# sndels/prosper

Measured on AMD Instinct MI355X. Metric: Mpaths/s, higher is better.
Workload: dtype f32; 1 GPU; S-cornell 1920x1080 8spp maxBounces 4; width=1920, height=1080, spp=8, max_bounces=4, triangles=38, bvh_nodes=7, parallelism=image stripes x1, pipeline=wavefront, 3 frames in flight (one launch chain each)

## Files before the change

### include/prosper_pt/prosper_pt.h

```cpp
#ifndef PROSPER_PT_H
#define PROSPER_PT_H

#include <stddef.h>
#include <stdint.h>

#include "shader_structs.h"

#ifdef __cplusplus
extern "C" {
#endif

#define PROSPER_PT_ABI_VERSION 4

enum
{
    PROSPER_PT_OK = 0,
    PROSPER_PT_ERR_INVALID_ARGUMENT = -1,
    PROSPER_PT_ERR_NO_DEVICE = -2,
    PROSPER_PT_ERR_HIP = -3,
    PROSPER_PT_ERR_NO_SCENE = -4,
    PROSPER_PT_ERR_SCENE = -5,
    PROSPER_PT_ERR_UNSUPPORTED = -6,
    PROSPER_PT_NOT_READY = -7,
};
// ... 119 lines not shown
    uint64_t pixelsWritten;
    uint64_t historyReads;
    uint64_t shortIndexHits;
    uint64_t shortIndexTriangleTests;
    uint64_t nodePhaseSteps;
    uint64_t trianglePhaseSteps;
    uint64_t anyHitTexelFetches;
} prosper_pt_counters;

typedef struct prosper_pt_scene_stats
{
    uint64_t triangleCount;
    uint64_t nodeCount;
    uint32_t nodeBytes;
    uint32_t triangleBytes;
    uint32_t maxDepth;
    uint32_t variantFlags;
    uint64_t deviceBytes;
    double buildSeconds;
    double uploadSeconds;
    double bvhBuildSeconds;
    double textureSeconds;
    uint64_t alphaTriangleCount;
    uint64_t alphaBoundBytes;
} prosper_pt_scene_stats;
enum
{
    PROSPER_PT_VARIANT_LDS_SCENE = 1u << 0,
    PROSPER_PT_VARIANT_LDS_TABLES = 1u << 1,
    PROSPER_PT_VARIANT_BATCHED_TEXTURES = 1u << 2,
    PROSPER_PT_VARIANT_TEXTURE_PACKS = 1u << 3,
    PROSPER_PT_VARIANT_RAW_RECORDS = 1u << 4,
    PROSPER_PT_VARIANT_STACK_SHIFT = 8,
};

enum
{
    PROSPER_PT_RENDER_COUNT_WORK = 1u << 0,
    PROSPER_PT_RENDER_PIPELINED = 1u << 1,
};

typedef struct prosper_pt_debug_options
{
    uint32_t struct_size;
    int32_t batchedTextures;
    int32_t widePacks;
    int32_t alphaCellShift;
    uint32_t noTexturePacks;
    uint32_t noAlphaBounds;
    uint32_t noUploadRefit;
    uint32_t flatBvh;
    float sahTraversalCost;
    float boxPad;
    uint32_t leafSize;
    uint32_t buildThreads;
    uint32_t topEntries;
    int32_t nodeOrder;
    int32_t childOrder;
    uint32_t buildTiming;
    uint32_t segments;
    uint32_t segmentLength;
    uint32_t chains;
    uint32_t ldsStackEntries;
    uint32_t noLdsScene;
    uint32_t noLdsTables;
    uint32_t traceDeadPaths;
    int32_t bandedBatches;
    float rebuildCostRatio;
    uint32_t alwaysRebuild;
    uint32_t failNextUpdate;
    uint32_t poolVariant;
    uint32_t rawRecords;
    uint32_t tileOrder;
    uint32_t hipGraph;
    uint32_t pipelinedChains;
    uint32_t mergeLimit;
} prosper_pt_debug_options;

const char *prosper_pt_last_error(void);
uint32_t prosper_pt_abi_version(void);
uint32_t prosper_pt_has_experiments(void);
void prosper_pt_debug_options_default(prosper_pt_debug_options *out);
int prosper_pt_set_debug_options(prosper_pt_ctx *ctx, const prosper_pt_debug_options *options);
int prosper_pt_get_debug_options(prosper_pt_ctx *ctx, prosper_pt_debug_options *out);

int prosper_pt_create(const prosper_pt_device_desc *desc, prosper_pt_ctx **out_ctx);
void prosper_pt_destroy(prosper_pt_ctx *ctx);

int prosper_pt_upload_scene(prosper_pt_ctx *ctx, const prosper_pt_scene_view *scene);
int prosper_pt_update_lights(
    prosper_pt_ctx *ctx, const prosper_DirectionalLightParameters *directionalLight,
    const prosper_PointLightsBuffer *pointLights, const prosper_SpotLightsBuffer *spotLights);
int prosper_pt_update_transforms(prosper_pt_ctx *ctx, const prosper_ModelInstanceTransforms *transforms, uint32_t count);
enum
{
    PROSPER_PT_UPDATE_NOW = 1u << 0,
};
int prosper_pt_update_transforms_async(
    prosper_pt_ctx *ctx, const prosper_ModelInstanceTransforms *transforms, uint32_t count, uint32_t flags, void *stream);
#define PROSPER_PT_ANIMATION_NONE 0xFFFFFFFFu
enum
{
    PROSPER_PT_NODE_HAS_TRANSLATION = 1u << 0,
    PROSPER_PT_NODE_HAS_ROTATION = 1u << 1,
    PROSPER_PT_NODE_HAS_SCALE = 1u << 2,
    PROSPER_PT_NODE_DIRECTIONAL_LIGHT = 1u << 3,
    PROSPER_PT_NODE_CAMERA = 1u << 4,
};
enum
{
    PROSPER_PT_ANIMATION_PATH_TRANSLATION = 0,
    PROSPER_PT_ANIMATION_PATH_ROTATION = 1,
    PROSPER_PT_ANIMATION_PATH_SCALE = 2,
};
enum
{
    PROSPER_PT_ANIMATION_STEP = 0,
// ... 706 lines not shown
```

### prosper_amd/capi.py

```python
import ctypes as C
import os
import subprocess

import numpy as np

from . import structs as S

_HERE = os.path.dirname(os.path.abspath(__file__))
LIB_PATH = os.environ.get("PROSPER_PT_LIB") or os.path.join(_HERE, "libprosper_pt.so")


class ProsperPtError(RuntimeError):
    def __init__(self, code, message):
        super().__init__("prosper_pt error %d: %s" % (code, message))
        self.code = code


def build(force=False):
    args = ["make", "-C", os.path.join(_HERE, "csrc"), "-s"]
    if force:
        args.append("-B")
    subprocess.check_call(args)
    return LIB_PATH


_lib = None


def lib():
    global _lib
    if _lib is not None:
        return _lib
    if not os.path.exists(LIB_PATH):
        raise ProsperPtError(-2, "HIP extension %s is missing: run prosper_amd.capi.build()" % LIB_PATH)
    L = C.CDLL(LIB_PATH)
    vp, u32, i32 = C.c_void_p, C.c_uint32, C.c_int32
    L.prosper_pt_last_error.restype = C.c_char_p
    L.prosper_pt_abi_version.restype = u32
    L.prosper_pt_has_experiments.restype = u32
    L.prosper_pt_debug_options_default.argtypes = [C.POINTER(S.DebugOptions)]
    L.prosper_pt_debug_options_default.restype = None
    L.prosper_pt_set_debug_options.argtypes = [vp, C.POINTER(S.DebugOptions)]
    L.prosper_pt_get_debug_options.argtypes = [vp, C.POINTER(S.DebugOptions)]
    L.prosper_pt_create.argtypes = [C.POINTER(S.DeviceDesc), C.POINTER(vp)]
    L.prosper_pt_destroy.argtypes = [vp]
    L.prosper_pt_destroy.restype = None
    L.prosper_pt_upload_scene.argtypes = [vp, C.POINTER(S.SceneView)]
    L.prosper_pt_update_lights.argtypes = [
        vp, C.POINTER(S.DirectionalLightParameters), C.POINTER(S.PointLightsBuffer), C.POINTER(S.SpotLightsBuffer)]
    L.prosper_pt_get_scene_stats.argtypes = [vp, C.POINTER(S.SceneStats)]
    L.prosper_pt_update_textures.argtypes = [vp, vp, u32, u32]
    L.prosper_pt_update_materials.argtypes = [vp, vp, u32, u32]
    L.prosper_pt_texture_mip_level_count.argtypes = [u32, u32]
    L.prosper_pt_texture_mip_level_count.restype = u32
    L.prosper_pt_check_texture_desc.argtypes = [C.POINTER(S.TextureDesc), u32]
    L.prosper_pt_get_texture_mips_info.argtypes = [vp, u32, C.POINTER(S.TextureMipsInfo)]
    L.prosper_pt_read_texture_level.argtypes = [vp, u32, u32, vp, C.c_uint64, vp]
    L.prosper_pt_debug_sample_texture_lod.argtypes = [vp, u32, u32, vp, u32, C.c_float, vp]
    L.prosper_pt_set_texture_lod.argtypes = [vp, C.c_int, C.c_float]
    L.prosper_pt_set_texture_lod_debug.argtypes = [vp, C.c_int]
    L.prosper_pt_read_texture_lod_derivatives.argtypes = [vp, vp, C.c_size_t, vp]
    L.prosper_pt_update_meshes.argtypes = [vp, vp, u32]
    L.prosper_pt_finish_mesh_updates.argtypes = [vp]
    L.prosper_pt_update_transforms.argtypes = [vp, vp, u32]
    L.prosper_pt_update_transforms_async.argtypes = [vp, vp, u32, u32, vp]
    L.prosper_pt_set_animations.argtypes = [vp, C.POINTER(S.AnimationDesc)]
    L.prosper_pt_animate.argtypes = [vp, C.c_float, u32, vp]
    L.prosper_pt_get_animation_state.argtypes = [vp, C.POINTER(S.AnimationStateInfo)]
    L.prosper_pt_read_animated_transforms.argtypes = [vp, u32, vp, u32]
    L.prosper_pt_read_lights.argtypes = [
        vp, C.POINTER(S.DirectionalLightParameters), C.POINTER(S.PointLightsBuffer), C.POINTER(S.SpotLightsBuffer)]
    L.prosper_pt_debug_read_animation_nodes.argtypes = [vp, vp, vp, u32]
    L.prosper_pt_rebuild_hierarchy.argtypes = [vp]
    L.prosper_pt_get_hierarchy_state.argtypes = [vp, C.POINTER(S.HierarchyState)]
    L.prosper_pt_debug_read_nodes.argtypes = [vp, vp, C.c_size_t]
    L.prosper_pt_set_output_buffer.argtypes = [vp, vp, C.c_size_t]
# ... 331 lines not shown
    rg, b = np.empty(2 * half_width, np.float32), np.empty(2 * half_width, np.float32)
    lib().prosper_pt_bloom_streak_weights(half_width, rg.ctypes.data, b.ctypes.data)
    return rg, b


def bloom_fft_plan(width, height, resolution_scale=0):
    plan = S.BloomFftPlan()
    _check(lib().prosper_pt_bloom_fft_plan(width, height, resolution_scale, C.byref(plan)))
    return plan


def has_experiments():
    return bool(lib().prosper_pt_has_experiments())


_debug_defaults = {}
_debug_version = 0


def debug(**options):
    global _debug_version
    if not options:
        _debug_defaults.clear()
    for k, v in options.items():
        if k not in dict(S.DebugOptions._fields_):
            raise KeyError("unknown debug option %r" % k)
        if v is None:
            _debug_defaults.pop(k, None)
        else:
            _debug_defaults[k] = v
    _debug_version += 1


class Context:

    def __init__(self, device=0, flags=0, _borrowed=None):
        self._owned = _borrowed is None
        self._own_debug = {}
        self._base_debug = None
        self._debug_seen = -1
        self._world = None
        self._animation_nodes = 0
        self._restir_extent = None
        if _borrowed is not None:
            self._h = C.c_void_p(_borrowed)
            return
        desc = S.DeviceDesc(C.sizeof(S.DeviceDesc), device, flags, 0)
        h = C.c_void_p()
        _check(lib().prosper_pt_create(C.byref(desc), C.byref(h)))
        self._h = h

    def set_debug(self, **options):
        if not options:
            self._own_debug = {}
        for k, v in options.items():
            if k not in dict(S.DebugOptions._fields_):
                raise KeyError("unknown debug option %r" % k)
            if v is None:
                self._own_debug.pop(k, None)
            else:
                self._own_debug[k] = v
        self._debug_seen = -1
        self._sync_debug()

    def debug_options(self):
        o = S.DebugOptions()
# ... 834 lines not shown
```

### prosper_amd/csrc/prosper_pt.cpp

```cpp
#include "../../include/prosper_pt/prosper_pt.h"

#include <hip/hip_runtime.h>

#include <algorithm>
#include <chrono>
#include <future>
#include <memory>
#include <cmath>
#include <cstdlib>
#include <cstdio>
#include <cstring>
#include <exception>
#include <stdexcept>
#include <string>
#include <vector>

#include "bvh_build.hpp"
#include "pt_animation.hpp"
#include "pt_context.hpp"
#include "pt_geometry.hpp"
#include "pt_kernels.hpp"
#include "pt_materials.hpp"
#include "pt_pass_support.hpp"
#include "pt_scene.hpp"
// ... 51 lines not shown
    if (bytes) PPT_HIP(hipMemcpy(*out, src, bytes, hipMemcpyHostToDevice));
    return PROSPER_PT_OK;
}

int grow_buffer(DeviceBuffer &buf, GrowWait wait, hipStream_t s, size_t bytes, size_t allocBytes, int fill)
{
    hipError_t e = hipSuccess;
    if (wait == GrowWait::Stream) e = hipStreamSynchronize(s);
    if (wait == GrowWait::Device) e = hipDeviceSynchronize();
    if (buf.ptr)
    {
        const hipError_t f = hipFree(buf.ptr);
        if (e == hipSuccess) e = f;
    }
    buf.ptr = nullptr;
    buf.bytes = 0;
    if (e == hipSuccess) e = hipMalloc(&buf.ptr, allocBytes);
    if (e == hipSuccess && fill >= 0) e = hipMemset(buf.ptr, fill, allocBytes);
    if (e != hipSuccess)
    {
        if (buf.ptr) (void)hipFree(buf.ptr);
        buf.ptr = nullptr;
        return fail(PROSPER_PT_ERR_HIP, std::string("growing a device buffer: ") + hipGetErrorString(e));
    }
    buf.bytes = bytes;
    return PROSPER_PT_OK;
}

}

namespace
{

WavefrontOptions wavefront_options(const prosper_pt_ctx *ctx)
{
    const prosper_pt_debug_options &d = ctx->debug;
    WavefrontOptions o;
    o.ldsStackEntries = d.ldsStackEntries;
    o.noLdsScene = d.noLdsScene != 0;
    o.noLdsTables = d.noLdsTables != 0;
    return o;
}

}

namespace
{

void free_scene(prosper_pt_ctx *ctx)
{
    discard_mesh_build(ctx);
    for (ppt::AccelState *old : ctx->retiredAccel) delete old;
    ctx->retiredAccel.clear();
    for (auto &a : ctx->sceneAllocations) (void)hipFree(a.ptr);
    ctx->sceneAllocations.clear();
    delete ctx->accel;
    ctx->accel = nullptr;
    delete ctx->lights;
    ctx->lights = nullptr;
    delete ctx->materialState;
    ctx->materialState = nullptr;
    delete ctx->geometry;
    ctx->geometry = nullptr;
    ctx->dTransforms = nullptr;
    ctx->sceneBytes = 0;
    ctx->haveScene = false;
    ctx->scene = DeviceScene{};
    ctx->textureMips = nullptr;
}

int validate_scene(const prosper_pt_scene_view *v, bool mips)
{
    if (v->struct_size != sizeof(prosper_pt_scene_view))
        return fail(PROSPER_PT_ERR_INVALID_ARGUMENT, "scene view struct_size mismatch");
    if (v->geometryBufferCount && (!v->geometryBuffers || !v->geometryBufferByteSizes))
// ... 1081 lines not shown
    out->nodeCount = acc->nodeCount;
    out->levels = (uint32_t)acc->levelOffsets.size() - 1u;
    return PROSPER_PT_OK;
}

int prosper_pt_debug_read_nodes(prosper_pt_ctx *ctx, void *out, size_t byte_size)
{
    if (!ctx || !out) return fail(PROSPER_PT_ERR_INVALID_ARGUMENT, "prosper_pt_debug_read_nodes: null argument");
    if (!ctx->haveScene || !ctx->accel) return fail(PROSPER_PT_ERR_NO_SCENE, "no scene uploaded");
    const size_t bytes = (size_t)ctx->accel->nodeCount * sizeof(BvhNode);
    if (byte_size < bytes) return fail(PROSPER_PT_ERR_INVALID_ARGUMENT, "prosper_pt_debug_read_nodes: destination too small");
    PPT_HIP(hipSetDevice(ctx->device));
    {
        const int frc = flush_pending_update(ctx, nullptr);
        if (frc != PROSPER_PT_OK) return frc;
    }
    PPT_HIP(hipDeviceSynchronize());
    PPT_HIP(hipMemcpy(out, ctx->accel->dNodes, bytes, hipMemcpyDeviceToHost));
    return PROSPER_PT_OK;
}

int prosper_pt_get_scene_stats(prosper_pt_ctx *ctx, prosper_pt_scene_stats *out)
{
    if (!ctx || !out) return fail(PROSPER_PT_ERR_INVALID_ARGUMENT, "prosper_pt_get_scene_stats: null argument");
    if (!ctx->haveScene) return fail(PROSPER_PT_ERR_NO_SCENE, "no scene uploaded");
    *out = ctx->stats;
    const WavefrontPlan plan = wavefront_plan(
        ctx->stats.maxDepth, (uint32_t)ctx->stats.nodeCount, (uint32_t)ctx->stats.triangleCount, ctx->scene, wavefront_options(ctx));
    const uint32_t ldsEntries = plan.ldsStackEntries;
    out->variantFlags =
        (plan.sceneInLds ? PROSPER_PT_VARIANT_LDS_SCENE : 0u) | (plan.tablesInLds ? PROSPER_PT_VARIANT_LDS_TABLES : 0u) |
        (ctx->scene.batchedTextures ? PROSPER_PT_VARIANT_BATCHED_TEXTURES : 0u) |
        (ctx->packedMaterials ? PROSPER_PT_VARIANT_TEXTURE_PACKS : 0u) |
        (ldsEntries << PROSPER_PT_VARIANT_STACK_SHIFT);
    return PROSPER_PT_OK;
}

int prosper_pt_set_output_buffer(prosper_pt_ctx *ctx, void *device_rgba32f, size_t byte_size)
{
    if (!ctx) return fail(PROSPER_PT_ERR_INVALID_ARGUMENT, "prosper_pt_set_output_buffer: null context");
    if (device_rgba32f && (reinterpret_cast<uintptr_t>(device_rgba32f) & 15u))
        return fail(PROSPER_PT_ERR_INVALID_ARGUMENT, "output buffer must be 16-byte aligned");
    ctx->externalHdr = device_rgba32f;
    ctx->externalHdrBytes = device_rgba32f ? byte_size : 0;
    return PROSPER_PT_OK;
}

static int render_wavefront(
    prosper_pt_ctx *ctx, const RenderParams &p, bool countWork, bool pipelined, uint32_t slotIndex, LaunchTimeline *tp,
    hipStream_t s)
{
    const uint32_t tilesX = (p.localWidth + 7u) / 8u, tilesY = (p.height + 7u) / 8u;
    const uint64_t pixelsPadded = (uint64_t)tilesX * tilesY * 64u;
    constexpr uint64_t kMaxWavefrontSlots = 64ull << 20;
    if (pixelsPadded > kMaxWavefrontSlots) return fail(PROSPER_PT_ERR_UNSUPPORTED, "image too large for the wavefront workspace");
    uint32_t framesPerChunk = (uint32_t)(kMaxWavefrontSlots / pixelsPadded);
    if (framesPerChunk > p.frameCount) framesPerChunk = p.frameCount;
    RenderSlot &slot = ctx->slots[slotIndex];
    ctx->lastSlot = slotIndex;
    WavefrontChains chains;
    chains.count = (pipelined || (ctx->flags & PROSPER_PT_CREATE_SINGLE_CHAIN)) ? 1u : 2u;
    if (!pipelined && ctx->debug.chains >= 1u && ctx->debug.chains <= kMaxChains) chains.count = ctx->debug.chains;
    chains.detached = pipelined;
    chains.fork = &ctx->chainFork;
    for (uint32_t i = 0; i < kMaxChains; ++i)
    {
        chains.streams[i] = ctx->workStreams[pipelined ? slotIndex : i].get();
// ... 351 lines not shown
```

### prosper_amd/csrc/pt_kernels.hpp

```cpp
#pragma once

#include <hip/hip_runtime.h>

#include "pt_scene.hpp"
#include "pt_sync.hpp"

namespace ppt
{

enum : uint32_t
{
    kStageGenerate = 0,
    kStageShade = 1,
    kStageTrace = 2,
    kStageAccumulate = 3,
    kStageCount = 4,
};

void launch_flatten_triangles(
    const DeviceScene &s, const uint32_t *triOffsets, uint32_t drawInstanceCount, const uint32_t *drawInstanceFlags,
    WorldTriangle *out, ShadeTriangle *shadeOut, AlphaTriangle *alphaOut, uint32_t total, hipStream_t stream,
    const uint32_t *leafPosition = nullptr, WorldTriangle *leafOrder = nullptr);
void launch_refit(
    BvhNode *nodes, const WorldTriangle *tris, float4 *bounds, const uint32_t *order, const uint32_t *levelOffsets,
// ... 2 lines not shown
    const DeviceTexture &tex, uint32_t wrapS, uint32_t wrapT, float factorA, uint32_t shift, uint16_t *out, hipStream_t stream);
void launch_srgb_monotonicity(uint32_t firstBits, uint32_t lastBits, uint32_t *out, hipStream_t stream);
void launch_permute_triangles(
    const WorldTriangle *in, const uint32_t *permutation, WorldTriangle *out, uint32_t total, hipStream_t stream);
void launch_tone_map(
    const float4 *hdr, const uint32_t *lut, uint32_t dim, float exposure, float contrast, void *outRgba8, uint32_t count,
    hipStream_t stream);
uint32_t megakernel_grid_blocks(const RenderParams &p);
uint32_t wavefront_grid_blocks(const WavefrontBuffers &w);
void launch_render_megakernel(
    const DeviceScene &s, const RenderParams &p, float4 *hdr, unsigned long long *counters, int32_t *stackOverflow,
    bool countWork, hipStream_t stream);
constexpr uint32_t kMaxChains = 3;
struct WavefrontChains
{
    uint32_t count = 1;
    bool detached = false;
    hipEvent_t after = nullptr;
    hipEvent_t scene = nullptr;
    hipEvent_t lights = nullptr;
    hipEvent_t materials = nullptr;
    hipStream_t streams[kMaxChains] = {};
    Fence *fork = nullptr;
    Fence *join[kMaxChains] = {};
    LaunchTimeline *timers[kMaxChains] = {};
};
struct WavefrontPlan
{
    uint32_t ldsStackEntries;
    uint32_t overflowEntries;
    bool sceneInLds;
    bool tablesInLds;
    uint32_t scratchDwordsPerBlock;
};
struct WavefrontOptions
{
    uint32_t ldsStackEntries = 0;
    bool noLdsScene = false, noLdsTables = false;
};
WavefrontPlan wavefront_plan(
    uint32_t stackBound, uint32_t nodeCount, uint32_t triCount, const DeviceScene &s, const WavefrontOptions &opt);
void launch_render_wavefront(
    const DeviceScene &s, const RenderParams &p, float4 *hdr, unsigned long long *counters, const WavefrontBuffers &w,
    const WavefrontPlan &plan, int32_t *scratch, uint32_t nodeCount, uint32_t triCount, bool countWork, LaunchTimeline *timer,
    const WavefrontChains &chains, hipStream_t stream);
uint32_t wavefront_lds_stack_entries(uint32_t stackBound, uint32_t forced);
bool wavefront_shade_tables_in_lds(const DeviceScene &s, bool disabled);
bool wavefront_scene_in_lds(uint32_t ldsStackEntries, uint32_t stackBound, uint32_t nodeCount, uint32_t triCount, bool disabled);
void launch_blit_rgba16f(const float4 *in, void *out, uint32_t count, hipStream_t stream);
constexpr uint32_t kMaxRanks = 64;
struct TileLayout
{
    uint32_t width, height, stripeWidth, ranks;
    uint32_t localWidth[kMaxRanks];
    uint64_t tileOffset[kMaxRanks];
};
void launch_deinterleave_tiles(const float4 *tiles, const TileLayout &layout, float4 *full, hipStream_t stream);
void launch_decode_bc7(
    const void *blocks, uint32_t width, uint32_t height, uint32_t tilesPerRow, void *tiled, hipStream_t stream);
void launch_retile_rgba8(const void *linear, uint32_t width, uint32_t height, uint32_t tilesPerRow, void *tiled, hipStream_t stream);
void launch_patch_alpha_records(AlphaTriangle *records, uint32_t count, const AlphaMaterial *table, uint32_t materialCount, hipStream_t stream);
void launch_border_skybox(const uint16_t *cube, uint32_t faceSize, void *bordered, hipStream_t stream);
void launch_pack_material_textures(
    const DeviceTexture &base, const DeviceTexture &mr, const DeviceTexture &normal, const MaterialPack &pack, hipStream_t stream);
void launch_eval_fn(
    uint32_t fn, const float *in, uint32_t inStride, float *out, uint32_t outStride, uint32_t n, hipStream_t stream);

}
```

### prosper_amd/csrc/pt_wavefront.hip

```cpp
#include "pt_kernels.hpp"

#include "pt_device.hpp"
#include "pt_render_common.hpp"
#include "pt_trace_stream.hpp"

#define PPT_SHADE_WPE 4
#ifndef PPT_GEN_WPE
#define PPT_GEN_WPE 5
#endif
#ifndef PPT_TRACE_WPE
#define PPT_TRACE_WPE(stack) 5
#endif

namespace ppt
{

namespace
{

constexpr uint32_t kSlotMask = 0x0FFFFFFFu;

struct SegmentId
{
    uint32_t seg;
// ... 210 lines not shown
    const BvhNode *gn = s.nodes;
    float *lf = reinterpret_cast<float *>(lds);
    for (uint32_t i = threadIdx.x; i < nodeCount * (kLdsNodeStride * 4u); i += blockDim.x)
    {
        const uint32_t n = i / (kLdsNodeStride * 4u), k = i - n * (kLdsNodeStride * 4u);
        const uint32_t q = k >> 2, c = k & 3u;
        float v = 0.0f;
        if (q == 0u)
            v = c < 3u ? gn[n].origin[c] : 0.0f;
        else if (q >= 1u && q <= 3u)
            v = half_to_float(gn[n].lo[q - 1u][c]);
        else if (q == 4u)
            v = __builtin_bit_cast(float, gn[n].child[c]);
        else if (q <= 7u)
            v = half_to_float(gn[n].hi[q - 5u][c]);
        lf[i] = v;
    }
    float4 *lt = lds + nodeCount * kLdsNodeStride;
    const float4 *gt = reinterpret_cast<const float4 *>(s.triangles);
    for (uint32_t i = threadIdx.x; i < triCount * 3u; i += blockDim.x) lt[i] = gt[i];
    __syncthreads();
    return LdsGeom{lds, lt};
}

}


template <bool COUNT, int STACK, bool LDS_SCENE>
__global__ __launch_bounds__(256, PPT_GEN_WPE) void wf_generate_extend(
    DeviceScene s, RenderParams p, WavefrontBuffers w, uint32_t nodeCount, uint32_t triCount,
    int32_t *__restrict__ stackOverflow, unsigned long long *__restrict__ counters)
{
    __shared__ int32_t ldsStack[STACK * 256];
    __shared__ float4 ldsScene[LDS_SCENE ? kLdsSceneFloat4s : 1];
    LdsGeomHalf lg = {};
    if constexpr (LDS_SCENE) lg = stage_scene_in_lds_half(s, ldsScene, nodeCount, triCount);
    const GlobalGeom gg{s.nodes, s.triangles};
    const SegmentId id = my_segment(w);
    if (!id.valid) return;
    const uint32_t lane = lane_id();
    const TraversalStack stack{(lds_int32 *)ldsStack + (threadIdx.x >> 6) * (STACK * 64u) + lane,
                               stackOverflow + blockIdx.x * 256u + threadIdx.x, (uint32_t)STACK, gridDim.x * 256u, 64u, LDS_SCENE};
    const bool traceRays = p.pc.maxBounces > 0;

    LaneCounters cnt = {};
    uint32_t nHit = 0;
    if (!traceRays)
    {
        for (uint32_t k = lane; k < w.segLen; k += 64u)
        {
            const SlotPixel sp = decode_slot(w, p, id.base + k);
            if (sp.valid)
            {
                if constexpr (COUNT) cnt.paths++;
                w.color[id.base + k] = make_float4(0.0f, 0.0f, 0.0f, 0.0f);
            }
        }
    }
    else
    {
        BatchLane bl = {};
        auto fetch = [&](uint32_t k) {
            const uint32_t at = id.base + k;
            StreamRay r;
            if (!bl.valid)
            {
                r.o = f3{0.0f, 0.0f, 0.0f};
// ... 281 lines not shown
        r.tMin = 0.1f;
        r.tMax = b.w;
        r.seed = asu(a.w);
        return r;
    };
    auto commit = [&](bool pred, uint32_t k, bool occluded, const Hit &, const f3 &) {
        if (pred)
        {
            const float4 c = sld(&w.shC[id.base + k]);
            const uint32_t packed = asu(c.w);
            const uint32_t nanMask = packed >> 28;
            if (!occluded || nanMask)
            {
                f3 v = xyz(c);
                if (occluded)
                {
                    const float nan = __builtin_nanf("");
                    v = f3{(nanMask & 1u) ? nan : 0.0f, (nanMask & 2u) ? nan : 0.0f, (nanMask & 4u) ? nan : 0.0f};
                }
                add_to_slot(w.color, packed & kSlotMask, p.pc.flags, v, bounce);
            }
        }
    };
    trace_stream<true, COUNT>(g, s, n, stack, cnt, fetch, commit);
}

template <bool COUNT, int STACK, bool LDS_SCENE>
__global__ __launch_bounds__(256, PPT_TRACE_WPE(STACK)) void wf_trace(
    DeviceScene s, RenderParams p, WavefrontBuffers w, uint32_t bounce, uint32_t nextCur, uint32_t doExtend,
    uint32_t nodeCount, uint32_t triCount, int32_t *__restrict__ stackOverflow,
    unsigned long long *__restrict__ counters)
{
    __shared__ int32_t ldsStack[STACK * 256];
    __shared__ float4 ldsScene[LDS_SCENE ? kLdsSceneFloat4s : 1];
    LdsGeom lg = {};
    if constexpr (LDS_SCENE) lg = stage_scene_in_lds(s, ldsScene, nodeCount, triCount);
    const GlobalGeom gg{s.nodes, s.triangles};
    const SegmentId id = my_segment(w);
    if (!id.valid) return;
    const TraversalStack stack{(lds_int32 *)ldsStack + (threadIdx.x >> 6) * (STACK * 64u) + lane_id(),
                               stackOverflow + blockIdx.x * 256u + threadIdx.x, (uint32_t)STACK, gridDim.x * 256u, 64u, LDS_SCENE};
    LaneCounters cnt = {};
    const uint32_t nShadow = w.segShadow[id.seg];
    const uint32_t nRays = doExtend ? w.segRays[id.seg] : 0u;
    if constexpr (LDS_SCENE)
        shadow_segment<COUNT>(lg, s, p, w, id, nShadow, bounce, stack, cnt);
    else
        shadow_segment<COUNT>(gg, s, p, w, id, nShadow, bounce, stack, cnt);
    if (doExtend)
    {
        __threadfence_block();
        uint32_t nHit;
        if constexpr (LDS_SCENE)
            nHit = extend_segment<COUNT>(lg, s, p, w, id, nRays, bounce + 1u, nextCur, stack, cnt);
        else
            nHit = extend_segment<COUNT>(gg, s, p, w, id, nRays, bounce + 1u, nextCur, stack, cnt);
        if (lane_id() == 0u) w.segHits[id.seg] = nHit;
    }
    flush_counters<COUNT>(cnt, counters);
}


template <bool COUNT>
__global__ __launch_bounds__(256) void wf_accumulate(
    RenderParams p, WavefrontBuffers w, float4 *__restrict__ hdr, unsigned long long *__restrict__ counters)
{
    const uint32_t rem = blockIdx.x * blockDim.x + threadIdx.x;
// ... 25 lines not shown
                const float invHc = 1.0f / hc;
                history = make_float4(
                    __builtin_fmaf(c.x - history.x, invHc, history.x), __builtin_fmaf(c.y - history.y, invHc, history.y),
                    __builtin_fmaf(c.z - history.z, invHc, history.z), hc);
                }
                if constexpr (COUNT) cnt.pixelsWritten++;
            }
            *texel = history;
        }
    }
    flush_counters<COUNT>(cnt, counters);
}


template <bool COUNT, int STACK, bool LDS_SCENE>
static void enqueue_wavefront(
    const DeviceScene &s, const RenderParams &p, unsigned long long *counters, const WavefrontBuffers &w,
    const WavefrontPlan &plan, uint32_t nodeCount, uint32_t triCount, int32_t *stackOverflow, LaunchTimeline *timer,
    hipStream_t stream)
{
    unsigned long long *cGen = counters + kStageGenerate * kCounterCount, *cShade = counters + kStageShade * kCounterCount,
                       *cTrace = counters + kStageTrace * kCounterCount;
    auto mark = [&](uint32_t st) {
        if (timer) timer->mark(st, stream);
    };
    const dim3 grid(((w.groupCount + 7u) / 8u) * 8u), block(256);
    uint32_t bounces = p.pc.maxBounces < PROSPER_RT_MAX_BOUNCES ? p.pc.maxBounces : PROSPER_RT_MAX_BOUNCES;
    const bool debugDraw =
        p.pc.drawType != PROSPER_DRAW_TYPE_DEFAULT && p.pc.drawType != PROSPER_DRAW_TYPE_MESHLET_ID;
    if (debugDraw && bounces > 1) bounces = 1;

    mark(kStageGenerate);
    hipLaunchKernelGGL(
        (wf_generate_extend<COUNT, STACK, LDS_SCENE>), grid, block, 0, stream, s, p, w, nodeCount, triCount,
        stackOverflow, cGen);
    for (uint32_t b = 0; b < bounces; ++b)
    {
        const uint32_t cur = b & 1u;
        const uint32_t last = (b + 1u == bounces) ? 1u : 0u;
        mark(kStageShade);
        const int ldsTables = !plan.tablesInLds ? 0 : (shade_table_bytes(s, true) <= kLdsTableBytes ? 1 : 2);
        auto shade = [&](auto kernel) { hipLaunchKernelGGL(kernel, grid, block, 0, stream, s, p, w, b, cur, last, cShade); };
        if (s.batchedTextures)
            ldsTables == 1 ? shade(wf_shade<COUNT, 1, true>) : (ldsTables == 2 ? shade(wf_shade<COUNT, 2, true>) : shade(wf_shade<COUNT, 0, true>));
        else
            ldsTables == 1 ? shade(wf_shade<COUNT, 1, false>) : (ldsTables == 2 ? shade(wf_shade<COUNT, 2, false>) : shade(wf_shade<COUNT, 0, false>));
        if (!debugDraw)
        {
            mark(kStageTrace);
            hipLaunchKernelGGL(
                (wf_trace<COUNT, STACK, LDS_SCENE>), grid, block, 0, stream, s, p, w, b, cur ^ 1u, last ? 0u : 1u,
                nodeCount, triCount, stackOverflow, cTrace);
        }
    }
}

uint32_t wavefront_grid_blocks(const WavefrontBuffers &w)
{
    const uint32_t groups = (w.nSeg + 3u) / 4u;
    return ((groups + 7u) / 8u) * 8u + 8u * kMaxChains;
}

uint32_t wavefront_lds_stack_entries(uint32_t stackBound, uint32_t forced)
{
    if (forced == 16u || forced == 24u || forced == 32u) return forced;
    return stackBound <= 16u ? 16u : 24u;
}

bool wavefront_shade_tables_in_lds(const DeviceScene &s, bool disabled)
{
    return shade_table_bytes(s, false) <= kLdsTableBytes && !disabled;
}
bool wavefront_scene_in_lds(uint32_t ldsStackEntries, uint32_t stackBound, uint32_t nodeCount, uint32_t triCount, bool disabled)
{
    return ldsStackEntries == 16u && stackBound <= 16u && nodeCount * kLdsNodeStride + triCount * 3u <= kLdsSceneFloat4s && !disabled;
}

WavefrontPlan wavefront_plan(
    uint32_t stackBound, uint32_t nodeCount, uint32_t triCount, const DeviceScene &s, const WavefrontOptions &opt)
{
    WavefrontPlan plan = {};
    plan.ldsStackEntries = wavefront_lds_stack_entries(stackBound, opt.ldsStackEntries);
    plan.overflowEntries = stackBound > plan.ldsStackEntries ? stackBound - plan.ldsStackEntries : 0u;
    plan.sceneInLds = wavefront_scene_in_lds(plan.ldsStackEntries, stackBound, nodeCount, triCount, opt.noLdsScene);
    plan.tablesInLds = wavefront_shade_tables_in_lds(s, opt.noLdsTables);
    plan.scratchDwordsPerBlock = plan.overflowEntries * 256u;
    return plan;
}

template <bool COUNT>
static void enqueue_for_stack(
    const DeviceScene &s, const RenderParams &p, unsigned long long *counters, const WavefrontBuffers &w,
    const WavefrontPlan &plan, int32_t *stackOverflow, uint32_t nodeCount, uint32_t triCount, LaunchTimeline *timer,
    hipStream_t stream)
{
    if (plan.sceneInLds)
        enqueue_wavefront<COUNT, 16, true>(s, p, counters, w, plan, nodeCount, triCount, stackOverflow, timer, stream);
    else if (plan.ldsStackEntries == 16u)
        enqueue_wavefront<COUNT, 16, false>(s, p, counters, w, plan, nodeCount, triCount, stackOverflow, timer, stream);
    else if (plan.ldsStackEntries == 24u)
        enqueue_wavefront<COUNT, 24, false>(s, p, counters, w, plan, nodeCount, triCount, stackOverflow, timer, stream);
    else
        enqueue_wavefront<COUNT, 32, false>(s, p, counters, w, plan, nodeCount, triCount, stackOverflow, timer, stream);
}

void launch_render_wavefront(
    const DeviceScene &s, const RenderParams &p, float4 *hdr, unsigned long long *counters, const WavefrontBuffers &w,
    const WavefrontPlan &plan, int32_t *stackOverflow, uint32_t nodeCount, uint32_t triCount, bool countWork,
    LaunchTimeline *timer, const WavefrontChains &chains, hipStream_t stream)
{
    if (w.nSeg == 0) return;
    static_assert(kTraversalStackDepth == 32, "largest LDS stack variant");
    const uint32_t groups = (w.nSeg + 3u) / 4u;
    uint32_t parts = chains.count < kMaxChains ? chains.count : kMaxChains;
    while (parts > 1u && groups < 256u * parts) --parts;
    const bool ownStreams = parts > 1u || chains.detached;
    const uint32_t per = (groups + parts - 1u) / parts;
    const bool forked = parts > 1u && !chains.detached;
    if (forked) (void)chains.fork->record(stream);
    uint32_t blocksBefore = 0;
    for (uint32_t i = 0; i < parts; ++i)
    {
        WavefrontBuffers part = w;
        part.groupBase = i * per;
        part.groupCount = (part.groupBase + per <= groups) ? per : groups - part.groupBase;
        hipStream_t cs = ownStreams ? chains.streams[i] : stream;
        LaunchTimeline *ct = ownStreams ? chains.timers[i] : timer;
        if (forked) (void)chains.fork->wait(cs);
        if (chains.detached && chains.after) (void)hipStreamWaitEvent(cs, chains.after, 0);
// ... 27 lines not shown
```

### prosper_amd/structs.py

```python
import ctypes as C

import numpy as np


class Vec4(C.Structure):
    _fields_ = [("x", C.c_float), ("y", C.c_float), ("z", C.c_float), ("w", C.c_float)]


class Mat4(C.Structure):
    _fields_ = [("col", Vec4 * 4)]


class Mat3x4(C.Structure):
    _fields_ = [("col", Vec4 * 3)]


class ReferencePC(C.Structure):

    _fields_ = [
        ("drawType", C.c_uint32),
        ("flags", C.c_uint32),
        ("frameIndex", C.c_uint32),
        ("apertureDiameter", C.c_float),
        ("focusDistance", C.c_float),
# ... 285 lines not shown
class DebugOptions(C.Structure):

    _fields_ = [("struct_size", C.c_uint32),
                ("batchedTextures", C.c_int32), ("widePacks", C.c_int32), ("alphaCellShift", C.c_int32),
                ("noTexturePacks", C.c_uint32), ("noAlphaBounds", C.c_uint32), ("noUploadRefit", C.c_uint32), ("flatBvh", C.c_uint32),
                ("sahTraversalCost", C.c_float), ("boxPad", C.c_float), ("leafSize", C.c_uint32), ("buildThreads", C.c_uint32),
                ("topEntries", C.c_uint32), ("nodeOrder", C.c_int32), ("childOrder", C.c_int32), ("buildTiming", C.c_uint32),
                ("segments", C.c_uint32), ("segmentLength", C.c_uint32), ("chains", C.c_uint32), ("ldsStackEntries", C.c_uint32),
                ("noLdsScene", C.c_uint32), ("noLdsTables", C.c_uint32), ("traceDeadPaths", C.c_uint32), ("bandedBatches", C.c_int32),
                ("rebuildCostRatio", C.c_float), ("alwaysRebuild", C.c_uint32), ("failNextUpdate", C.c_uint32),
                ("poolVariant", C.c_uint32), ("rawRecords", C.c_uint32), ("tileOrder", C.c_uint32), ("hipGraph", C.c_uint32),
                ("pipelinedChains", C.c_uint32), ("mergeLimit", C.c_uint32)]


class CommInfo(C.Structure):
    _fields_ = [("ranks", C.c_uint32), ("rank", C.c_uint32), ("device", C.c_int32), ("gathers", C.c_uint32),
                ("lastGatherMs", C.c_float), ("reserved", C.c_uint32)]


class MeshUpdate(C.Structure):
    _fields_ = [("meshIndex", C.c_uint32), ("reserved", C.c_uint32), ("metadata", GeometryMetadata), ("info", MeshInfo),
                ("bytes", C.c_void_p), ("byteOffset", C.c_uint64), ("byteCount", C.c_uint64), ("bufferByteSize", C.c_uint64)]


MAX_GEOMETRY_BUFFERS = 100
GATHER_IN_STREAM = 1
UPDATE_NOW = 1
VARIANT_LDS_SCENE = 1
VARIANT_LDS_TABLES = 2
VARIANT_BATCHED_TEXTURES = 4
VARIANT_TEXTURE_PACKS = 8
VARIANT_RAW_RECORDS = 16
VARIANT_STACK_SHIFT = 8


def as_numpy(struct_array, dtype=np.uint8):
    return np.frombuffer(struct_array, dtype=dtype)


class RestirTracePC(C.Structure):
    _fields_ = [("drawType", C.c_uint32), ("frameIndex", C.c_uint32), ("flags", C.c_uint32)]


class RestirInputs(C.Structure):
    _fields_ = [("albedoRoughness", C.c_void_p), ("normalMetallic", C.c_void_p), ("nonLinearDepth", C.c_void_p),
                ("reservoirs", C.c_void_p), ("onDevice", C.c_uint32), ("reserved", C.c_uint32)]


RESTIR_INITIAL = 0
RESTIR_SPATIAL = 1
RESTIR_SPATIAL_REUSE = 1

RESTIR_TRACE_GBUFFER = 1 << 1
RESTIR_JITTER_GBUFFER = 1 << 2
GBUFFER_JITTER = 1 << 0
GBUFFER_OPAQUE_ONLY = 1 << 2


class GBufferTargets(C.Structure):
    _fields_ = [("albedoRoughness", C.c_void_p), ("normalMetallic", C.c_void_p), ("nonLinearDepth", C.c_void_p)]


class VelocityGBufferDesc(C.Structure):
    _fields_ = [("targets", GBufferTargets), ("velocity", C.c_void_p), ("previousTransforms", C.c_void_p),
                ("previousTransformCount", C.c_uint32)]

# ... 233 lines not shown
```

Measured before the change: 8885 Mpaths/s.

## Size LDS scene dynamically and shrink LDS stack when scene fits in LDS

Replaces the fixed-size static LDS scene array in the generate and trace kernels with dynamic shared memory sized to the actual node and triangle count. When the scene is staged in LDS, it also chooses a smaller LDS traversal stack (8 or 12 entries) based on the stack bound, with new template instantiations for those sizes. The aim is to cut LDS use per block so more trace workgroups fit on each CU. A debug API reports the resulting plan. The risk is that a smaller stack or altered occupancy may not help if traversal is not bound by occupancy.

```diff
diff --git a/include/prosper_pt/prosper_pt.h b/include/prosper_pt/prosper_pt.h
--- a/include/prosper_pt/prosper_pt.h
+++ b/include/prosper_pt/prosper_pt.h
@@ -175,6 +175,8 @@
     PROSPER_PT_VARIANT_TEXTURE_PACKS = 1u << 3,
     PROSPER_PT_VARIANT_RAW_RECORDS = 1u << 4,
     PROSPER_PT_VARIANT_STACK_SHIFT = 8,
+    PROSPER_PT_VARIANT_WAVES_SHIFT = 16,
+    PROSPER_PT_VARIANT_LDS_SHIFT = 20,
 };
 
 enum
@@ -226,6 +228,20 @@
 void prosper_pt_debug_options_default(prosper_pt_debug_options *out);
 int prosper_pt_set_debug_options(prosper_pt_ctx *ctx, const prosper_pt_debug_options *options);
 int prosper_pt_get_debug_options(prosper_pt_ctx *ctx, prosper_pt_debug_options *out);
+typedef struct prosper_pt_traversal_plan
+{
+    uint32_t ldsStackEntries;
+    uint32_t sceneInLds;
+    uint32_t traceWaves;
+    uint32_t sceneLdsBytes;
+    uint32_t traceLdsBytes;
+    uint32_t groupsPerCu;
+    uint32_t cuLdsBytes;
+    uint32_t reserved;
+} prosper_pt_traversal_plan;
+int prosper_pt_debug_traversal_plan(
+    uint32_t stackBound, uint32_t nodeCount, uint32_t triangleCount, const prosper_pt_debug_options *options,
+    prosper_pt_traversal_plan *out);
 
 int prosper_pt_create(const prosper_pt_device_desc *desc, prosper_pt_ctx **out_ctx);
 void prosper_pt_destroy(prosper_pt_ctx *ctx);
diff --git a/prosper_amd/capi.py b/prosper_amd/capi.py
--- a/prosper_amd/capi.py
+++ b/prosper_amd/capi.py
@@ -42,6 +42,7 @@
     L.prosper_pt_debug_options_default.restype = None
     L.prosper_pt_set_debug_options.argtypes = [vp, C.POINTER(S.DebugOptions)]
     L.prosper_pt_get_debug_options.argtypes = [vp, C.POINTER(S.DebugOptions)]
+    L.prosper_pt_debug_traversal_plan.argtypes = [u32, u32, u32, C.POINTER(S.DebugOptions), C.POINTER(S.TraversalPlan)]
     L.prosper_pt_create.argtypes = [C.POINTER(S.DeviceDesc), C.POINTER(vp)]
     L.prosper_pt_destroy.argtypes = [vp]
     L.prosper_pt_destroy.restype = None
@@ -439,6 +440,18 @@
     _debug_version += 1
 
 
+def traversal_plan(stack_bound, node_count, triangle_count, **options):
+    o = S.DebugOptions()
+    lib().prosper_pt_debug_options_default(C.byref(o))
+    for k, v in options.items():
+        if k not in dict(S.DebugOptions._fields_):
+            raise KeyError("unknown debug option %r" % k)
+        setattr(o, k, v)
+    out = S.TraversalPlan()
+    _check(lib().prosper_pt_debug_traversal_plan(stack_bound, node_count, triangle_count, C.byref(o), C.byref(out)))
+    return out
+
+
 class Context:
 
     def __init__(self, device=0, flags=0, _borrowed=None):
diff --git a/prosper_amd/csrc/prosper_pt.cpp b/prosper_amd/csrc/prosper_pt.cpp
--- a/prosper_amd/csrc/prosper_pt.cpp
+++ b/prosper_amd/csrc/prosper_pt.cpp
@@ -107,15 +107,15 @@
 namespace
 {
 
-WavefrontOptions wavefront_options(const prosper_pt_ctx *ctx)
-{
-    const prosper_pt_debug_options &d = ctx->debug;
+WavefrontOptions wavefront_options(const prosper_pt_debug_options &d)
+{
     WavefrontOptions o;
     o.ldsStackEntries = d.ldsStackEntries;
     o.noLdsScene = d.noLdsScene != 0;
     o.noLdsTables = d.noLdsTables != 0;
     return o;
 }
+WavefrontOptions wavefront_options(const prosper_pt_ctx *ctx) { return wavefront_options(ctx->debug); }
 
 }
 
@@ -1263,7 +1263,36 @@
         (plan.sceneInLds ? PROSPER_PT_VARIANT_LDS_SCENE : 0u) | (plan.tablesInLds ? PROSPER_PT_VARIANT_LDS_TABLES : 0u) |
         (ctx->scene.batchedTextures ? PROSPER_PT_VARIANT_BATCHED_TEXTURES : 0u) |
         (ctx->packedMaterials ? PROSPER_PT_VARIANT_TEXTURE_PACKS : 0u) |
-        (ldsEntries << PROSPER_PT_VARIANT_STACK_SHIFT);
+        (ldsEntries << PROSPER_PT_VARIANT_STACK_SHIFT) | (plan.traceWaves << PROSPER_PT_VARIANT_WAVES_SHIFT) |
+        ((plan.traceLdsBytes / 16u) << PROSPER_PT_VARIANT_LDS_SHIFT);
+    return PROSPER_PT_OK;
+}
+
+int prosper_pt_debug_traversal_plan(
+    uint32_t stackBound, uint32_t nodeCount, uint32_t triangleCount, const prosper_pt_debug_options *options,
+    prosper_pt_traversal_plan *out)
+{
+    if (!out) return fail(PROSPER_PT_ERR_INVALID_ARGUMENT, "prosper_pt_debug_traversal_plan: null argument");
+    prosper_pt_debug_options o;
+    prosper_pt_debug_options_default(&o);
+    if (options)
+    {
+        if (options->struct_size != sizeof(prosper_pt_debug_options))
+            return fail(PROSPER_PT_ERR_INVALID_ARGUMENT, "prosper_pt_debug_traversal_plan: struct_size mismatch");
+        const int rc = check_debug_options(*options);
+        if (rc != PROSPER_PT_OK) return rc;
+        o = *options;
+    }
+    const DeviceScene none = {};
+    const WavefrontPlan plan = wavefront_plan(stackBound, nodeCount, triangleCount, none, wavefront_options(o));
+    *out = {};
+    out->ldsStackEntries = plan.ldsStackEntries;
+    out->sceneInLds = plan.sceneInLds ? 1u : 0u;
+    out->traceWaves = plan.traceWaves;
+    out->sceneLdsBytes = plan.traceSceneLdsBytes;
+    out->traceLdsBytes = plan.traceLdsBytes;
+    out->groupsPerCu = plan.traceGroupsPerCu;
+    out->cuLdsBytes = kCuLdsBytes;
     return PROSPER_PT_OK;
 }
 
diff --git a/prosper_amd/csrc/pt_kernels.hpp b/prosper_amd/csrc/pt_kernels.hpp
--- a/prosper_amd/csrc/pt_kernels.hpp
+++ b/prosper_amd/csrc/pt_kernels.hpp
@@ -58,12 +58,20 @@
     bool sceneInLds;
     bool tablesInLds;
     uint32_t scratchDwordsPerBlock;
+    uint32_t traceWaves;
+    uint32_t traceSceneLdsBytes;
+    uint32_t genSceneLdsBytes;
+    uint32_t traceLdsBytes;
+    uint32_t traceGroupsPerCu;
 };
 struct WavefrontOptions
 {
     uint32_t ldsStackEntries = 0;
     bool noLdsScene = false, noLdsTables = false;
 };
+constexpr uint32_t kCuLdsBytes = 160u * 1024u, kLdsGranuleBytes = 1280u;
+uint32_t wavefront_lds_groups_per_cu(uint32_t ldsBytes);
+uint32_t wavefront_trace_lds_bytes(uint32_t stackEntries, uint32_t sceneBytes);
 WavefrontPlan wavefront_plan(
     uint32_t stackBound, uint32_t nodeCount, uint32_t triCount, const DeviceScene &s, const WavefrontOptions &opt);
 void launch_render_wavefront(
diff --git a/prosper_amd/csrc/pt_wavefront.hip b/prosper_amd/csrc/pt_wavefront.hip
--- a/prosper_amd/csrc/pt_wavefront.hip
+++ b/prosper_amd/csrc/pt_wavefront.hip
@@ -266,7 +266,7 @@
     int32_t *__restrict__ stackOverflow, unsigned long long *__restrict__ counters)
 {
     __shared__ int32_t ldsStack[STACK * 256];
-    __shared__ float4 ldsScene[LDS_SCENE ? kLdsSceneFloat4s : 1];
+    extern __shared__ float4 ldsScene[];
     LdsGeomHalf lg = {};
     if constexpr (LDS_SCENE) lg = stage_scene_in_lds_half(s, ldsScene, nodeCount, triCount);
     const GlobalGeom gg{s.nodes, s.triangles};
@@ -614,7 +614,7 @@
     unsigned long long *__restrict__ counters)
 {
     __shared__ int32_t ldsStack[STACK * 256];
-    __shared__ float4 ldsScene[LDS_SCENE ? kLdsSceneFloat4s : 1];
+    extern __shared__ float4 ldsScene[];
     LdsGeom lg = {};
     if constexpr (LDS_SCENE) lg = stage_scene_in_lds(s, ldsScene, nodeCount, triCount);
     const GlobalGeom gg{s.nodes, s.triangles};
@@ -706,8 +706,8 @@
 
     mark(kStageGenerate);
     hipLaunchKernelGGL(
-        (wf_generate_extend<COUNT, STACK, LDS_SCENE>), grid, block, 0, stream, s, p, w, nodeCount, triCount,
-        stackOverflow, cGen);
+        (wf_generate_extend<COUNT, STACK, LDS_SCENE>), grid, block, LDS_SCENE ? plan.genSceneLdsBytes : 0u, stream, s, p, w,
+        nodeCount, triCount, stackOverflow, cGen);
     for (uint32_t b = 0; b < bounces; ++b)
     {
         const uint32_t cur = b & 1u;
@@ -723,8 +723,8 @@
         {
             mark(kStageTrace);
             hipLaunchKernelGGL(
-                (wf_trace<COUNT, STACK, LDS_SCENE>), grid, block, 0, stream, s, p, w, b, cur ^ 1u, last ? 0u : 1u,
-                nodeCount, triCount, stackOverflow, cTrace);
+                (wf_trace<COUNT, STACK, LDS_SCENE>), grid, block, LDS_SCENE ? plan.traceSceneLdsBytes : 0u, stream, s, p, w, b,
+                cur ^ 1u, last ? 0u : 1u, nodeCount, triCount, stackOverflow, cTrace);
         }
     }
 }
@@ -750,15 +750,31 @@
     return ldsStackEntries == 16u && stackBound <= 16u && nodeCount * kLdsNodeStride + triCount * 3u <= kLdsSceneFloat4s && !disabled;
 }
 
+uint32_t wavefront_lds_groups_per_cu(uint32_t ldsBytes)
+{
+    const uint32_t granules = (ldsBytes + kLdsGranuleBytes - 1u) / kLdsGranuleBytes;
+    return granules == 0u ? ~0u : (kCuLdsBytes / kLdsGranuleBytes) / granules;
+}
+uint32_t wavefront_trace_lds_bytes(uint32_t stackEntries, uint32_t sceneBytes) { return stackEntries * 256u * 4u + sceneBytes; }
+
 WavefrontPlan wavefront_plan(
     uint32_t stackBound, uint32_t nodeCount, uint32_t triCount, const DeviceScene &s, const WavefrontOptions &opt)
 {
     WavefrontPlan plan = {};
     plan.ldsStackEntries = wavefront_lds_stack_entries(stackBound, opt.ldsStackEntries);
+    plan.sceneInLds = wavefront_scene_in_lds(plan.ldsStackEntries, stackBound, nodeCount, triCount, opt.noLdsScene);
+    plan.traceWaves = PPT_TRACE_WPE(16);
+    if (plan.sceneInLds)
+    {
+        if (opt.ldsStackEntries == 0u) plan.ldsStackEntries = stackBound <= 8u ? 8u : (stackBound <= 12u ? 12u : 16u);
+        plan.traceSceneLdsBytes = (nodeCount * kLdsNodeStride + triCount * 3u) * 16u;
+        plan.genSceneLdsBytes = (nodeCount * kLdsNodeStrideHalf + triCount * 3u) * 16u;
+    }
     plan.overflowEntries = stackBound > plan.ldsStackEntries ? stackBound - plan.ldsStackEntries : 0u;
-    plan.sceneInLds = wavefront_scene_in_lds(plan.ldsStackEntries, stackBound, nodeCount, triCount, opt.noLdsScene);
     plan.tablesInLds = wavefront_shade_tables_in_lds(s, opt.noLdsTables);
     plan.scratchDwordsPerBlock = plan.overflowEntries * 256u;
+    plan.traceLdsBytes = wavefront_trace_lds_bytes(plan.ldsStackEntries, plan.traceSceneLdsBytes);
+    plan.traceGroupsPerCu = wavefront_lds_groups_per_cu(plan.traceLdsBytes);
     return plan;
 }
 
@@ -768,7 +784,11 @@
     const WavefrontPlan &plan, int32_t *stackOverflow, uint32_t nodeCount, uint32_t triCount, LaunchTimeline *timer,
     hipStream_t stream)
 {
-    if (plan.sceneInLds)
+    if (plan.sceneInLds && plan.ldsStackEntries == 8u)
+        enqueue_wavefront<COUNT, 8, true>(s, p, counters, w, plan, nodeCount, triCount, stackOverflow, timer, stream);
+    else if (plan.sceneInLds && plan.ldsStackEntries == 12u)
+        enqueue_wavefront<COUNT, 12, true>(s, p, counters, w, plan, nodeCount, triCount, stackOverflow, timer, stream);
+    else if (plan.sceneInLds)
         enqueue_wavefront<COUNT, 16, true>(s, p, counters, w, plan, nodeCount, triCount, stackOverflow, timer, stream);
     else if (plan.ldsStackEntries == 16u)
         enqueue_wavefront<COUNT, 16, false>(s, p, counters, w, plan, nodeCount, triCount, stackOverflow, timer, stream);
diff --git a/prosper_amd/structs.py b/prosper_amd/structs.py
--- a/prosper_amd/structs.py
+++ b/prosper_amd/structs.py
@@ -341,6 +341,25 @@
 VARIANT_TEXTURE_PACKS = 8
 VARIANT_RAW_RECORDS = 16
 VARIANT_STACK_SHIFT = 8
+VARIANT_WAVES_SHIFT = 16
+VARIANT_LDS_SHIFT = 20
+
+
+def variant_stack_entries(flags):
+    return (flags >> VARIANT_STACK_SHIFT) & 0xFF
+
+
+def variant_trace_waves(flags):
+    return (flags >> VARIANT_WAVES_SHIFT) & 0xF
+
+
+def variant_trace_lds_bytes(flags):
+    return (flags >> VARIANT_LDS_SHIFT) * 16
+
+
+class TraversalPlan(C.Structure):
+    _fields_ = [("ldsStackEntries", C.c_uint32), ("sceneInLds", C.c_uint32), ("traceWaves", C.c_uint32), ("sceneLdsBytes", C.c_uint32),
+                ("traceLdsBytes", C.c_uint32), ("groupsPerCu", C.c_uint32), ("cuLdsBytes", C.c_uint32), ("reserved", C.c_uint32)]
 
 
 def as_numpy(struct_array, dtype=np.uint8):
```

Result: no change. 8910 Mpaths/s, median of 2 (+0.3%).
